# idiap/IdiapTTS

Hardware: AMD Instinct MI355X
Metric: acoustic frames/sec (train) (higher is better)
Workload: dtype f32

## Files before the change

### idiaptts_amd/csrc/sparse_rows.hip

```cpp
#include <algorithm>
#include <atomic>
#include <utility>

#include "activations.h"
#include "common.h"

namespace itts {

constexpr int kSparseMaxK = 512;
constexpr int kSlabCols = 64;
constexpr int kFwdWaves = 16;
constexpr int kRowsPerWave = 4;
constexpr int kStep = 8;
constexpr int kFetch = 16;

static std::atomic<int64_t> g_sparse_path[3];

struct ListLayout {
  int64_t counts_off, entries_off, pitch, bytes;
};

static ListLayout list_layout(int64_t M, int K) {
  ListLayout l;
  l.counts_off = 16;
  l.entries_off = 16 + (M * 4 + 15) / 16 * 16;
  l.pitch = ((int64_t)K + kFetch - 1) / kFetch * kFetch;
  l.bytes = l.entries_off + M * l.pitch * 8;
  return l;
}

__global__ __launch_bounds__(256) void sparse_rows_build_kernel(const uint32_t* __restrict__ x, int64_t ldx, int64_t M,
                                                                int K, int* __restrict__ counts,
                                                                int2* __restrict__ entries, int64_t pitch,
                                                                unsigned long long* __restrict__ record) {
  const int lane = threadIdx.x & 63;
  const int64_t w0 = (int64_t)blockIdx.x * 4 + (threadIdx.x >> 6), wn = (int64_t)gridDim.x * 4;
  const unsigned long long below = (1ull << lane) - 1ull;
  unsigned long long total = 0, most = 0;
  for (int64_t m = w0; m < M; m += wn) {
    const uint32_t* row = x + m * ldx;
    int2* out = entries + m * pitch;
    int cnt = 0;
    for (int k0 = 0; k0 < K; k0 += 256) {
      uint32_t bits[4];
#pragma unroll
      for (int u = 0; u < 4; ++u) {
        const int k = k0 + 64 * u + lane;
        bits[u] = k < K ? row[k] : 0u;
      }
#pragma unroll
      for (int u = 0; u < 4; ++u) {
        const bool nz = (bits[u] & 0x7fffffffu) != 0u;
        const unsigned long long mask = __ballot(nz);
        if (nz) out[cnt + __popcll(mask & below)] = make_int2(k0 + 64 * u + lane, (int)bits[u]);
        cnt += __popcll(mask);
      }
    }
    if (lane < ((kStep - cnt % kStep) % kStep)) out[cnt + lane] = make_int2(K, 0);
    if (lane == 0) counts[m] = cnt;
    total += (unsigned long long)cnt;
    most = std::max(most, (unsigned long long)cnt);
  }
  if (record && lane == 0 && total) {
    atomicAdd(&record[0], total);
    atomicMax(&record[1], most);
  }
}

template <int J>
__device__ __forceinline__ void walk_slot(const float4* slab4, int i16, int2 e, float4& acc) {
  const int k = __builtin_amdgcn_update_dpp(0, e.x, 0x150 + J, 0xf, 0xf, false);
  const float v = __int_as_float(__builtin_amdgcn_update_dpp(0, e.y, 0x150 + J, 0xf, 0xf, false));
  const float4 wk = slab4[k * (kSlabCols / 4) + i16];
  acc.x = fmaf(v, wk.x, acc.x); acc.y = fmaf(v, wk.y, acc.y);
  acc.z = fmaf(v, wk.z, acc.z); acc.w = fmaf(v, wk.w, acc.w);
}
template <int FIRST, int... U>
__device__ __forceinline__ void walk_trip(const float4* slab4, int i16, int2 e, float4& acc,
                                          std::integer_sequence<int, U...>) {
  (walk_slot<FIRST + U>(slab4, i16, e, acc), ...);
}

template <int AF>
__global__ __launch_bounds__(kFwdWaves * 64) void sparse_linear_fwd_kernel(
    const int* __restrict__ counts, const int2* __restrict__ entries, int64_t pitch, const float* __restrict__ w,
    const float* __restrict__ bias, float* __restrict__ y, int64_t ldy, int64_t M, int N, int K, int act, int ranges,
    int store_cols, int wide_out) {
  extern __shared__ float4 slab4[];
  float* slab = reinterpret_cast<float*>(slab4);
  const int lane = threadIdx.x & 63;
  const int wave = __builtin_amdgcn_readfirstlane((int)(threadIdx.x >> 6));
  const int n0 = (int)(blockIdx.x / ranges) * kSlabCols;
  const int range = (int)(blockIdx.x % ranges);
  const int64_t per = (M + ranges - 1) / ranges;
  const int64_t m_begin = range * per, m_end = std::min<int64_t>(M, m_begin + per);
  const int q = lane >> 4, c4 = (lane & 15) * 4;

  {
    const bool col_ok = n0 + lane < N;
    const float* wr = w + (int64_t)(col_ok ? n0 + lane : 0) * K;
    for (int k = wave; k < K; k += kFwdWaves) slab[k * kSlabCols + lane] = col_ok ? wr[k] : 0.f;
    if (wave == 0) slab[K * kSlabCols + lane] = 0.f;
  }

  auto row_of = [&](int64_t group) { return m_begin + (group * kRowsPerWave + q); };
  const int i16 = lane & 15;
  auto fetch = [&](int64_t m, int j0) { return entries[std::min<int64_t>(m, M - 1) * pitch + (j0 + i16)]; };
  int64_t group = wave;
  int2 first = fetch(row_of(group), 0);
  int cnt_next = counts[std::min<int64_t>(row_of(group), M - 1)];
  __syncthreads();

  float4 bv = make_float4(0.f, 0.f, 0.f, 0.f);
  const int n = n0 + c4;
  if (bias) {
    if (n < N) bv.x = bias[n];
    if (n + 1 < N) bv.y = bias[n + 1];
    if (n + 2 < N) bv.z = bias[n + 2];
    if (n + 3 < N) bv.w = bias[n + 3];
  }
  const bool vec_store = wide_out && n + 4 <= store_cols;
  const int last_fetch = (int)pitch - kFetch;

  for (; m_begin + group * kRowsPerWave < m_end; group += kFwdWaves) {
    const int64_t m = row_of(group);
    const int cnt = m < m_end ? cnt_next : 0;
    int2 cur = first;
    first = fetch(row_of(group + kFwdWaves), 0);
    cnt_next = counts[std::min<int64_t>(row_of(group + kFwdWaves), M - 1)];
    int longest = std::max(cnt, __shfl_xor(cnt, 16, 64));
    longest = __builtin_amdgcn_readfirstlane(std::max(longest, __shfl_xor(longest, 32, 64)));
    float4 acc = make_float4(0.f, 0.f, 0.f, 0.f);
    for (int j0 = 0; j0 < longest; j0 += kFetch) {
      const int2 nxt = fetch(m, std::min(j0 + kFetch, last_fetch));
      if (j0 < cnt) walk_trip<0>(slab4, i16, cur, acc, std::make_integer_sequence<int, kStep>());
      if (j0 + kStep < cnt) walk_trip<kStep>(slab4, i16, cur, acc, std::make_integer_sequence<int, kStep>());
      cur = nxt;
    }
    if (m < m_end) {
      float4 o;
      o.x = n < N ? act_fwd_af<AF>(acc.x + bv.x, act) : 0.f;
      o.y = n + 1 < N ? act_fwd_af<AF>(acc.y + bv.y, act) : 0.f;
      o.z = n + 2 < N ? act_fwd_af<AF>(acc.z + bv.z, act) : 0.f;
      o.w = n + 3 < N ? act_fwd_af<AF>(acc.w + bv.w, act) : 0.f;
      float* yr = y + m * ldy + n;
      if (vec_store) {
        *reinterpret_cast<float4*>(yr) = o;
      } else {
        if (n < store_cols) yr[0] = o.x;
        if (n + 1 < store_cols) yr[1] = o.y;
        if (n + 2 < store_cols) yr[2] = o.z;
        if (n + 3 < store_cols) yr[3] = o.w;
      }
    }
  }
}

}

using namespace itts;

extern "C" int itts_sparse_rows_layout(int64_t M, int K, int64_t out[4]) {
  ITTS_REQUIRE(out != nullptr, "null pointer");
  ITTS_REQUIRE(M >= 0 && K > 0 && K <= 65535, "bad sizes (K <= 65535)");
  const ListLayout l = list_layout(M, K);
  out[0] = l.counts_off; out[1] = l.entries_off; out[2] = l.pitch; out[3] = l.bytes;
  return ITTS_OK;
}

extern "C" int itts_sparse_rows_build(const float* d_x, int64_t ldx, int64_t M, int K, void* d_lists, int want_record,
                                      void* stream) {
  ITTS_REQUIRE(d_lists && (M == 0 || d_x), "null pointer");
  ITTS_REQUIRE(M >= 0 && K > 0 && K <= 65535 && ldx >= K, "bad sizes (K <= 65535)");
  ITTS_REQUIRE(aligned16(d_lists), "the list block must be 16-byte aligned");
  hipStream_t s = as_stream(stream);
  char* base = static_cast<char*>(d_lists);
  if (want_record) ITTS_HIP_CHECK(hipMemsetAsync(base, 0, 16, s));
  if (M == 0) return ITTS_OK;
  const ListLayout l = list_layout(M, K);
  const unsigned grid = (unsigned)std::min<int64_t>((M + 3) / 4, 8192);
  hipLaunchKernelGGL(sparse_rows_build_kernel, dim3(grid), dim3(256), 0, s, reinterpret_cast<const uint32_t*>(d_x), ldx,
                     M, K, reinterpret_cast<int*>(base + l.counts_off), reinterpret_cast<int2*>(base + l.entries_off),
                     l.pitch, want_record ? reinterpret_cast<unsigned long long*>(base) : nullptr);
  ITTS_LAUNCH_CHECK();
  g_sparse_path[0].fetch_add(1, std::memory_order_relaxed);
  return ITTS_OK;
}

static int fwd_compute_units() {
  static int cus = 0;
  if (cus == 0) {
    int dev = 0, n = 0;
    if (hipGetDevice(&dev) != hipSuccess ||
        hipDeviceGetAttribute(&n, hipDeviceAttributeMultiprocessorCount, dev) != hipSuccess || n <= 0)
      n = 256;
    cus = n;
  }
  return cus;
}

template <int AF>
static int launch_sparse_fwd(const void* d_lists, const float* d_w, const float* d_b, float* d_y, int64_t ldy, int64_t M,
                             int N, int K, int act, hipStream_t s) {
  static bool lds_set = false;
  if (!lds_set) {
    ITTS_HIP_CHECK(hipFuncSetAttribute((const void*)sparse_linear_fwd_kernel<AF>,
                                       hipFuncAttributeMaxDynamicSharedMemorySize,
                                       (kSparseMaxK + 1) * kSlabCols * 4));
    lds_set = true;
  }
  const ListLayout l = list_layout(M, K);
  const char* base = static_cast<const char*>(d_lists);
  const int slabs = (N + kSlabCols - 1) / kSlabCols;
  const int64_t ranges = std::max<int64_t>(1, std::min<int64_t>(fwd_compute_units() / slabs, (M + 63) / 64));
  const bool wide_out = (ldy % 4 == 0) && aligned16(d_y);
  const int store_cols = wide_out ? (int)std::min<int64_t>((N + 3) / 4 * 4, ldy) : N;
  hipLaunchKernelGGL(sparse_linear_fwd_kernel<AF>, dim3((unsigned)(slabs * ranges)), dim3(kFwdWaves * 64),
                     (size_t)(K + 1) * kSlabCols * 4, s, reinterpret_cast<const int*>(base + l.counts_off),
                     reinterpret_cast<const int2*>(base + l.entries_off), l.pitch, d_w, d_b, d_y, ldy, M, N, K, act,
                     (int)ranges, store_cols, wide_out ? 1 : 0);
  ITTS_LAUNCH_CHECK();
  return ITTS_OK;
}

extern "C" int itts_linear_fwd_sparse(const void* d_lists, const float* d_x, int64_t ldx, const float* d_w,
                                      const float* d_b, float* d_y, int64_t ldy, int64_t M, int N, int K, int act,
                                      void* stream) {
  ITTS_REQUIRE(d_w && (M == 0 || (d_lists && d_x && d_y)), "null pointer");
  ITTS_REQUIRE(M >= 0 && N > 0 && K > 0 && K <= 65535 && ldx >= K && ldy >= N, "bad sizes");
  ITTS_REQUIRE(act >= ITTS_ACT_NONE && act <= ITTS_ACT_HARDSIGMOID, "unknown activation");
  if (M == 0) return ITTS_OK;
  if (K > kSparseMaxK) {
    g_sparse_path[2].fetch_add(1, std::memory_order_relaxed);
    return itts_linear_fwd(d_x, ldx, d_w, d_b, d_y, ldy, M, N, K, act, stream);
  }
  g_sparse_path[1].fetch_add(1, std::memory_order_relaxed);
  if (act_family(act) == AF_EXT) return launch_sparse_fwd<AF_EXT>(d_lists, d_w, d_b, d_y, ldy, M, N, K, act, as_stream(stream));
  return launch_sparse_fwd<AF_BASE>(d_lists, d_w, d_b, d_y, ldy, M, N, K, act, as_stream(stream));
}

extern "C" int itts_sparse_path_counts(int64_t out[3]) {
  ITTS_REQUIRE(out != nullptr, "null pointer");
  for (int i = 0; i < 3; ++i) out[i] = g_sparse_path[i].load(std::memory_order_relaxed);
  return ITTS_OK;
}
```

### idiaptts_amd/csrc/sparse_wgrad.hip

```cpp
#include <algorithm>
#include <atomic>

#include "common.h"

namespace itts {

constexpr int kWgMaxK = 512;
constexpr int kTile = 256;
constexpr int kSlab = 64;
constexpr int kWgWaves = 16;
constexpr int kOwners = 64;
constexpr int kSlots = 8;
constexpr int kStrip = 32;
constexpr int kBlock = 16;
constexpr int kGroup = 4;
constexpr int kHeaderBytes = kSlots * 2;
constexpr int kFirstBytes = kBlock * 8;
constexpr int kOverBytes = (kTile / kBlock - 1) * kBlock * 8;
constexpr int kPlanInv = kStrip + kOwners * kSlots;
constexpr int kPlanInts = kPlanInv + kWgMaxK;
constexpr int kHeavyCode = 0x1000;
constexpr int kRowBytes = kSlab * 4;
constexpr int kBufBytes = (kTile + 1) * kRowBytes;
constexpr int kTPitch = 513;
constexpr int kBiasFloat = 2 * kBufBytes / 4;
constexpr int kWgLdsBytes = 2 * kBufBytes + kSlab * 4;
static_assert(kSlab * kTPitch * 4 <= 2 * kBufBytes, "the output tile reuses the dz buffers");

static std::atomic<int64_t> g_wgrad_path[3];

struct ColsLayout {
  int64_t tiles, strip_off, streams_off, bytes;
};

static ColsLayout cols_layout(int64_t M) {
  ColsLayout l;
  l.tiles = (M + kTile - 1) / kTile;
  l.strip_off = 0;
  l.streams_off = l.tiles * kTile * kStrip * 4;
  l.bytes = l.streams_off + l.tiles * kOwners * (int64_t)(kHeaderBytes + kSlots * (kFirstBytes + kOverBytes));
  return l;
}

__device__ __forceinline__ const char* firsts_of(const char* streams, int tiles) {
  return streams + (int64_t)tiles * kOwners * kHeaderBytes;
}
__device__ __forceinline__ const char* overs_of(const char* streams, int tiles) {
  return firsts_of(streams, tiles) + (int64_t)tiles * kOwners * kSlots * kFirstBytes;
}
__device__ __forceinline__ int2* entry_of(char* streams, int tiles, int64_t pair, int j) {
  char* p = j < kBlock ? const_cast<char*>(firsts_of(streams, tiles)) + pair * kFirstBytes + j * 8
                       : const_cast<char*>(overs_of(streams, tiles)) + pair * kOverBytes + (j - kBlock) * 8;
  return reinterpret_cast<int2*>(p);
}

__global__ __launch_bounds__(256) void sparse_cols_build_kernel(const uint32_t* __restrict__ x, int64_t ldx, int64_t M,
                                                                int K, int parts, int tiles,
                                                                const int* __restrict__ plan,
                                                                uint32_t* __restrict__ strip,
                                                                char* __restrict__ streams) {
  __shared__ int cnts[4][64];
  const int tile = (int)(blockIdx.x / (parts + 1)), part = (int)(blockIdx.x % (parts + 1));
  const int lane = threadIdx.x & 63, wave = threadIdx.x >> 6;
  const int64_t m0 = (int64_t)tile * kTile + wave * 64;
  if (part == parts) {
    const int h = lane & 31;
    const int hc = h < kStrip - 1 ? plan[h] : -1;
    if (!(hc >= 0 && hc < K)) {
      for (int i = 0; i < 32; ++i) {
        const int64_t m = m0 + 2 * i + (lane >> 5);
        strip[m * kStrip + h] = (m < M && h == kStrip - 1) ? 0x3f800000u : 0u;
      }
    }
    for (int pair = threadIdx.x; pair < kOwners * kSlots; pair += 256) {
      const int c = plan[kStrip + pair];
      if (!(c >= 0 && c < K))
        reinterpret_cast<uint16_t*>(streams + ((int64_t)tile * kOwners + pair / kSlots) * kHeaderBytes)[pair % kSlots] = 0;
    }
    return;
  }
  const int k = part * 64 + lane;
  const bool valid = k < K;
  const int code = valid ? plan[kPlanInv + k] : -1;
  const bool light = code >= 0 && code < kOwners * kSlots;
  const bool heavy = code >= kHeavyCode && code < kHeavyCode + kStrip - 1;
  uint32_t bits[64];
#pragma unroll
  for (int r = 0; r < 64; ++r) bits[r] = (valid && m0 + r < M) ? x[(m0 + r) * ldx + k] : 0u;
  int cnt = 0;
#pragma unroll
  for (int r = 0; r < 64; ++r) cnt += (bits[r] & 0x7fffffffu) != 0u ? 1 : 0;
  cnts[wave][lane] = cnt;
  __syncthreads();
  if (heavy) {
    uint32_t* dst = strip + m0 * kStrip + (code - kHeavyCode);
#pragma unroll
    for (int r = 0; r < 64; ++r) dst[r * kStrip] = bits[r];
  }
  if (!light) return;
  int before = 0, total = 0;
#pragma unroll
  for (int w = 0; w < 4; ++w) {
    const int c = cnts[w][lane];
    before += w < wave ? c : 0;
    total += c;
  }
  const int owner = code / kSlots, slot = code % kSlots;
  const int64_t pair = ((int64_t)tile * kOwners + owner) * kSlots + slot;
  int j = before;
#pragma unroll
  for (int r = 0; r < 64; ++r)
    if ((bits[r] & 0x7fffffffu) != 0u)
      *entry_of(streams, tiles, pair, j++) = make_int2((wave * 64 + r) * kRowBytes, (int)bits[r]);
  if (wave == 0) {
    const int end = (total + kBlock - 1) / kBlock * kBlock;
    for (int e = total; e < end; ++e) *entry_of(streams, tiles, pair, e) = make_int2(kTile * kRowBytes, 0);
    reinterpret_cast<uint16_t*>(streams + ((int64_t)tile * kOwners + owner) * kHeaderBytes)[slot] = (uint16_t)total;
  }
}

typedef float floatx16 __attribute__((ext_vector_type(16)));

template <int J>
__device__ __forceinline__ void col_slot(const char* buf, int lane_off, int2 e, float4& acc) {
  const int off = __builtin_amdgcn_update_dpp(0, e.x, 0x150 + J, 0xf, 0xf, false);
  const float v = __int_as_float(__builtin_amdgcn_update_dpp(0, e.y, 0x150 + J, 0xf, 0xf, false));
  const float4 d = *reinterpret_cast<const float4*>(buf + off + lane_off);
  acc.x = fmaf(v, d.x, acc.x); acc.y = fmaf(v, d.y, acc.y);
  acc.z = fmaf(v, d.z, acc.z); acc.w = fmaf(v, d.w, acc.w);
}
template <int FIRST>
__device__ __forceinline__ void col_group(const char* buf, int lane_off, int2 e, float4& acc) {
  col_slot<FIRST>(buf, lane_off, e, acc);
  col_slot<FIRST + 1>(buf, lane_off, e, acc);
  col_slot<FIRST + 2>(buf, lane_off, e, acc);
  col_slot<FIRST + 3>(buf, lane_off, e, acc);
}

__global__ __launch_bounds__(kWgWaves * 64) void sparse_wgrad_kernel(
    const float* __restrict__ dz, int64_t lddz, const float* __restrict__ strip, const char* __restrict__ streams,
    const int* __restrict__ plan, float* __restrict__ slabs, int64_t slab_stride, int lddw,
    float* __restrict__ bias_part, int64_t bias_stride, int64_t M, int N, int K, int tiles, int per, int ranges) {
  extern __shared__ float4 smem4[];
  char* smem = reinterpret_cast<char*>(smem4);
  float* smemf = reinterpret_cast<float*>(smem4);
  const int tid = threadIdx.x, lane = tid & 63;
  const int wave = __builtin_amdgcn_readfirstlane(tid >> 6);
  const int i16 = lane & 15, owner = wave * 4 + (lane >> 4);
  const int n0 = (int)(blockIdx.x / ranges) * kSlab;
  const int range = (int)(blockIdx.x % ranges);
  const int t_begin = range * per, t_end = std::min(tiles, t_begin + per);

  if (tid < 128) smemf[((tid >> 6) * kBufBytes + kTile * kRowBytes) / 4 + lane] = 0.f;

  const int srow = tid >> 4, c4 = (tid & 15) * 4, n = n0 + c4;
  auto load_tile = [&](int t, float4 (&st)[4]) {
#pragma unroll
    for (int p = 0; p < 4; ++p) {
      const int64_t m = (int64_t)t * kTile + p * 64 + srow;
      float4 v = make_float4(0.f, 0.f, 0.f, 0.f);
      if (m < M) {
        const float* src = dz + m * lddz + n;
        if (n + 4 <= N) {
          v = *reinterpret_cast<const float4*>(src);
        } else {
          if (n < N) v.x = src[0];
          if (n + 1 < N) v.y = src[1];
          if (n + 2 < N) v.z = src[2];
        }
      }
      st[p] = v;
    }
  };
  auto store_tile = [&](int b, const float4 (&st)[4]) {
#pragma unroll
    for (int p = 0; p < 4; ++p)
      *reinterpret_cast<float4*>(smem + b * kBufBytes + (p * 64 + srow) * kRowBytes + c4 * 4) = st[p];
  };
  const char* firsts = firsts_of(streams, tiles) + i16 * 8;
  const char* overs = overs_of(streams, tiles) + i16 * 8;
  auto lists_of = [&](int t) { return ((int64_t)t * kOwners + owner) * kSlots; };

  float4 acc[kSlots];
#pragma unroll
  for (int c = 0; c < kSlots; ++c) acc[c] = make_float4(0.f, 0.f, 0.f, 0.f);
  floatx16 hacc;
#pragma unroll
  for (int r = 0; r < 16; ++r) hacc[r] = 0.f;

  uint4 hdr;
  int2 first[kSlots];
  auto load_lists = [&](int t) {
    hdr = *reinterpret_cast<const uint4*>(streams + ((int64_t)t * kOwners + owner) * kHeaderBytes);
#pragma unroll
    for (int c = 0; c < kSlots; ++c)
      first[c] = *reinterpret_cast<const int2*>(firsts + (lists_of(t) + c) * kFirstBytes);
  };
  auto count_of = [&](int c) {
    const uint32_t word = c < 2 ? hdr.x : (c < 4 ? hdr.y : (c < 6 ? hdr.z : hdr.w));
    return (int)((word >> ((c & 1) * 16)) & 0xffffu);
  };

  float4 st[4];
  load_tile(t_begin, st);
  load_lists(t_begin);
  store_tile(0, st);
  __syncthreads();

  const int hb = wave >> 3, hr0 = (wave & 7) * 32 + (lane >> 5);
  for (int t = t_begin; t < t_end; ++t) {
    const int b = (t - t_begin) & 1;
    const int tn = std::min(t + 1, t_end - 1);
    const char* buf = smem + b * kBufBytes;
    const char* more = overs + lists_of(t) * kOverBytes;
    int2 over = first[0];
    if (count_of(0) > kBlock) over = *reinterpret_cast<const int2*>(more);
#pragma unroll
    for (int c = 0; c < kSlots; ++c) {
      const int cnt = count_of(c);
      int longest = std::max(cnt, __shfl_xor(cnt, 16, 64));
      longest = __builtin_amdgcn_readfirstlane(std::max(longest, __shfl_xor(longest, 32, 64)));
      int2 over_n = over;
      if (c + 1 < kSlots && count_of(c + 1 < kSlots ? c + 1 : c) > kBlock)
        over_n = *reinterpret_cast<const int2*>(more + (c + 1) * kOverBytes);
      int2 cur = first[c];
      for (int j0 = 0; j0 < longest; j0 += kBlock) {
        const int left = cnt - j0;
        if (left > 0) {
          int2 ahead = over;
          if (left > 2 * kBlock) ahead = *reinterpret_cast<const int2*>(more + c * kOverBytes + (j0 + kBlock) * 8);
          col_group<0>(buf, i16 * 16, cur, acc[c]);
          if (left > kGroup) col_group<kGroup>(buf, i16 * 16, cur, acc[c]);
          if (left > 2 * kGroup) col_group<2 * kGroup>(buf, i16 * 16, cur, acc[c]);
          if (left > 3 * kGroup) col_group<3 * kGroup>(buf, i16 * 16, cur, acc[c]);
          cur = over;
          over = ahead;
        }
      }
      over = over_n;
    }
    load_tile(tn, st);
    {
      const float* a = reinterpret_cast<const float*>(buf) + hr0 * kSlab + hb * 32 + (lane & 31);
      const float* xh = strip + ((int64_t)t * kTile + hr0) * kStrip + (lane & 31);
#pragma unroll
      for (int kk = 0; kk < 16; ++kk)
        hacc = __builtin_amdgcn_mfma_f32_32x32x2f32(a[2 * kk * kSlab], xh[2 * kk * kStrip], hacc, 0, 0, 0);
    }
    store_tile(b ^ 1, st);
    load_lists(tn);
    __syncthreads();
  }

  for (int i = tid; i < kBiasFloat + kSlab; i += kWgWaves * 64) smemf[i] = 0.f;
  __syncthreads();
#pragma unroll
  for (int c = 0; c < kSlots; ++c) {
    const int col = plan[kStrip + owner * kSlots + c];
    if (col >= 0 && col < K) {
      smemf[(4 * i16 + 0) * kTPitch + col] = acc[c].x;
      smemf[(4 * i16 + 1) * kTPitch + col] = acc[c].y;
      smemf[(4 * i16 + 2) * kTPitch + col] = acc[c].z;
      smemf[(4 * i16 + 3) * kTPitch + col] = acc[c].w;
    }
  }
  __syncthreads();
  {
    const int h = lane & 31;
    const int hc = h < kStrip - 1 ? plan[h] : -1;
    for (int w = 0; w < kWgWaves; ++w) {
      if (wave == w) {
#pragma unroll
        for (int r = 0; r < 16; ++r) {
          const int nl = hb * 32 + 8 * (r / 4) + 4 * (lane >> 5) + (r % 4);
          if (h == kStrip - 1) smemf[kBiasFloat + nl] += hacc[r];
          else if (hc >= 0 && hc < K) smemf[nl * kTPitch + hc] += hacc[r];
        }
      }
      __syncthreads();
    }
  }
  for (int nn = wave; nn < kSlab; nn += kWgWaves) {
    if (n0 + nn < N) {
      float* dst = slabs + range * slab_stride + (int64_t)(n0 + nn) * lddw;
      for (int k = lane; k < lddw; k += 64) dst[k] = smemf[nn * kTPitch + k];
    }
  }
  if (bias_part && tid < kSlab && n0 + tid < N)
    bias_part[range * bias_stride + n0 + tid] = smemf[kBiasFloat + tid];
}

static int wgrad_compute_units() {
  static int cus = 0;
  if (cus == 0) {
    int dev = 0, n = 0;
    if (hipGetDevice(&dev) != hipSuccess ||
        hipDeviceGetAttribute(&n, hipDeviceAttributeMultiprocessorCount, dev) != hipSuccess || n <= 0)
      n = 256;
    cus = n;
  }
  return cus;
}

static void wgrad_ranges(int64_t M, int N, int* per, int* ranges) {
  const int64_t tiles = (M + kTile - 1) / kTile;
  const int slabs = (N + kSlab - 1) / kSlab;
  const int64_t want = std::max<int64_t>(1, std::min<int64_t>(wgrad_compute_units() / slabs, tiles));
  *per = (int)((tiles + want - 1) / want);
  *ranges = (int)((tiles + *per - 1) / *per);
}

static bool wgrad_shape_ok(int K, int64_t lddw) { return K <= kWgMaxK && lddw <= kWgMaxK; }

}

using namespace itts;

extern "C" int itts_sparse_cols_plan_ints(void) { return kPlanInts; }

extern "C" int itts_sparse_cols_layout(int64_t M, int K, int64_t out[3]) {
  ITTS_REQUIRE(out != nullptr, "null pointer");
  ITTS_REQUIRE(M >= 0 && K > 0 && K <= kWgMaxK, "bad sizes (K <= 512)");
  const ColsLayout l = cols_layout(M);
  out[0] = l.strip_off; out[1] = l.streams_off; out[2] = l.bytes;
  return ITTS_OK;
}

extern "C" int itts_sparse_cols_build(const float* d_x, int64_t ldx, int64_t M, int K, const int* d_plan, void* d_cols,
                                      void* stream) {
  ITTS_REQUIRE(d_plan && d_cols && (M == 0 || d_x), "null pointer");
  ITTS_REQUIRE(M >= 0 && K > 0 && K <= kWgMaxK && ldx >= K, "bad sizes (K <= 512)");
  ITTS_REQUIRE(aligned16(d_cols), "the column block must be 16-byte aligned");
  if (M == 0) return ITTS_OK;
  const ColsLayout l = cols_layout(M);
  const int parts = (K + 63) / 64;
  ITTS_REQUIRE(l.tiles * (parts + 1) < ((int64_t)1 << 31), "too many rows");
  char* base = static_cast<char*>(d_cols);
  hipLaunchKernelGGL(sparse_cols_build_kernel, dim3((unsigned)(l.tiles * (parts + 1))), dim3(256), 0,
                     as_stream(stream), reinterpret_cast<const uint32_t*>(d_x), ldx, M, K, parts, (int)l.tiles, d_plan,
                     reinterpret_cast<uint32_t*>(base + l.strip_off), base + l.streams_off);
  ITTS_LAUNCH_CHECK();
  g_wgrad_path[0].fetch_add(1, std::memory_order_relaxed);
  return ITTS_OK;
}

extern "C" int64_t itts_linear_bwd_weight_sparse_workspace_bytes(int64_t M, int N, int K, int64_t lddw) {
  if (M < 0 || N <= 0 || K <= 0 || lddw < K) return 0;
  const int64_t dense = itts_linear_bwd_weight_workspace_bytes(M, N, (int)lddw);
  if (M == 0 || !wgrad_shape_ok(K, lddw)) return dense;
  int per, ranges;
  wgrad_ranges(M, N, &per, &ranges);
  return std::max<int64_t>(dense, (int64_t)ranges * ((int64_t)N * lddw + N) * 4);
}

extern "C" int itts_linear_bwd_weight_sparse(const float* d_dz, int64_t lddz, const void* d_cols, const int* d_plan,
                                             const float* d_x, int64_t ldx, float* d_dw, int64_t lddw, float* d_db,
                                             int64_t M, int N, int K, void* d_workspace, int accumulate,
                                             void* stream) {
  ITTS_REQUIRE(d_dw && d_workspace && (M == 0 || (d_dz && d_x)), "null pointer");
  ITTS_REQUIRE(M >= 0 && N > 0 && K > 0 && lddz >= N && ldx >= K && lddw >= K, "bad sizes");
  ITTS_REQUIRE(lddw == K || ldx >= lddw, "x must be as wide as dw's rows (its pad columns zero)");
  const bool sparse = M > 0 && d_cols && d_plan && wgrad_shape_ok(K, lddw) && lddz % 4 == 0 && aligned16(d_dz) &&
                      aligned16(d_cols);
  if (!sparse) {
    if (M > 0) g_wgrad_path[2].fetch_add(1, std::memory_order_relaxed);
    return itts_linear_bwd_weight(d_dz, lddz, d_x, ldx, d_dw, d_db, M, N, (int)lddw, d_workspace, accumulate, stream);
  }
  hipStream_t s = as_stream(stream);
  static bool lds_set = false;
  if (!lds_set) {
    ITTS_HIP_CHECK(hipFuncSetAttribute((const void*)sparse_wgrad_kernel, hipFuncAttributeMaxDynamicSharedMemorySize,
                                       kWgLdsBytes));
    lds_set = true;
  }
  const ColsLayout l = cols_layout(M);
  int per, ranges;
  wgrad_ranges(M, N, &per, &ranges);
  const int slabs_n = (N + kSlab - 1) / kSlab;
  ITTS_REQUIRE((int64_t)slabs_n * ranges < ((int64_t)1 << 31), "too many workgroups");
  const int64_t n = (int64_t)N * lddw;
  const bool merged = d_db && d_db == d_dw + n && N % 4 == 0 && n % 4 == 0;
  float* ws = static_cast<float*>(d_workspace);
  float* bias_part = !d_db ? nullptr : (merged ? ws + n : ws + (int64_t)ranges * n);
  const char* base = static_cast<const char*>(d_cols);
  hipLaunchKernelGGL(sparse_wgrad_kernel, dim3((unsigned)(slabs_n * ranges)), dim3(kWgWaves * 64), kWgLdsBytes, s, d_dz,
                     lddz, reinterpret_cast<const float*>(base + l.strip_off), base + l.streams_off, d_plan, ws,
                     merged ? n + N : n, (int)lddw, bias_part, merged ? n + N : (int64_t)N, M, N, K, (int)l.tiles, per,
                     ranges);
  ITTS_LAUNCH_CHECK();
  g_wgrad_path[1].fetch_add(1, std::memory_order_relaxed);
  if (merged) return reduce_slabs(ws, ranges, n + N, d_dw, accumulate, s);
  int rc = reduce_slabs(ws, ranges, n, d_dw, accumulate, s);
  if (rc || !d_db) return rc;
  return reduce_slabs(bias_part, ranges, (int64_t)N, d_db, accumulate, s);
}

extern "C" int itts_sparse_wgrad_counts(int64_t out[3]) {
  ITTS_REQUIRE(out != nullptr, "null pointer");
  for (int i = 0; i < 3; ++i) out[i] = g_wgrad_path[i].load(std::memory_order_relaxed);
  return ITTS_OK;
}
```

Baseline: 41.02 million.

## Vectorize sparse forward weight slab fill and parallelize wgrad hidden-tile reduction

The sparse forward kernel now loads weight rows as float4 when K is a multiple of four and the pointer is 16-byte aligned, then scatters the four values into the transposed LDS slab. The wgrad kernel replaces a sixteen-step serialized per-wave accumulation, which had a barrier per wave, with a staged LDS reduction. In that reduction each wave stores its MFMA accumulators, then sums two rows across the eight waves of its half-block and writes the result directly. This removes many block-wide barriers at the cost of extra LDS traffic and an assumption about how the hb groups are laid out across waves.

```diff
diff --git a/idiaptts_amd/csrc/sparse_rows.hip b/idiaptts_amd/csrc/sparse_rows.hip
--- a/idiaptts_amd/csrc/sparse_rows.hip
+++ b/idiaptts_amd/csrc/sparse_rows.hip
@@ -13,6 +13,7 @@
 constexpr int kRowsPerWave = 4;
 constexpr int kStep = 8;
 constexpr int kFetch = 16;
+constexpr int kFillTrips = kSparseMaxK / 4 / kFwdWaves;
 
 static std::atomic<int64_t> g_sparse_path[3];
 
@@ -85,7 +86,7 @@
 __global__ __launch_bounds__(kFwdWaves * 64) void sparse_linear_fwd_kernel(
     const int* __restrict__ counts, const int2* __restrict__ entries, int64_t pitch, const float* __restrict__ w,
     const float* __restrict__ bias, float* __restrict__ y, int64_t ldy, int64_t M, int N, int K, int act, int ranges,
-    int store_cols, int wide_out) {
+    int store_cols, int wide_out, int wide_w) {
   extern __shared__ float4 slab4[];
   float* slab = reinterpret_cast<float*>(slab4);
   const int lane = threadIdx.x & 63;
@@ -99,7 +100,26 @@
   {
     const bool col_ok = n0 + lane < N;
     const float* wr = w + (int64_t)(col_ok ? n0 + lane : 0) * K;
-    for (int k = wave; k < K; k += kFwdWaves) slab[k * kSlabCols + lane] = col_ok ? wr[k] : 0.f;
+    if (wide_w) {
+      const float4* wr4 = reinterpret_cast<const float4*>(wr);
+      const int K4 = K >> 2;
+      float4 v[kFillTrips];
+#pragma unroll
+      for (int u = 0; u < kFillTrips; ++u) {
+        const int j = wave + u * kFwdWaves;
+        v[u] = (col_ok && j < K4) ? wr4[j] : make_float4(0.f, 0.f, 0.f, 0.f);
+      }
+#pragma unroll
+      for (int u = 0; u < kFillTrips; ++u) {
+        const int j = wave + u * kFwdWaves;
+        if (j < K4) {
+          float* row = slab + 4 * j * kSlabCols + lane;
+          row[0] = v[u].x; row[kSlabCols] = v[u].y; row[2 * kSlabCols] = v[u].z; row[3 * kSlabCols] = v[u].w;
+        }
+      }
+    } else {
+      for (int k = wave; k < K; k += kFwdWaves) slab[k * kSlabCols + lane] = col_ok ? wr[k] : 0.f;
+    }
     if (wave == 0) slab[K * kSlabCols + lane] = 0.f;
   }
 
@@ -218,7 +238,7 @@
   hipLaunchKernelGGL(sparse_linear_fwd_kernel<AF>, dim3((unsigned)(slabs * ranges)), dim3(kFwdWaves * 64),
                      (size_t)(K + 1) * kSlabCols * 4, s, reinterpret_cast<const int*>(base + l.counts_off),
                      reinterpret_cast<const int2*>(base + l.entries_off), l.pitch, d_w, d_b, d_y, ldy, M, N, K, act,
-                     (int)ranges, store_cols, wide_out ? 1 : 0);
+                     (int)ranges, store_cols, wide_out ? 1 : 0, (K % 4 == 0 && aligned16(d_w)) ? 1 : 0);
   ITTS_LAUNCH_CHECK();
   return ITTS_OK;
 }
diff --git a/idiaptts_amd/csrc/sparse_wgrad.hip b/idiaptts_amd/csrc/sparse_wgrad.hip
--- a/idiaptts_amd/csrc/sparse_wgrad.hip
+++ b/idiaptts_amd/csrc/sparse_wgrad.hip
@@ -252,6 +252,22 @@
     __syncthreads();
   }
 
+  float hsum[2];
+  {
+#pragma unroll
+    for (int r = 0; r < 16; ++r) smemf[(wave * 16 + r) * 64 + lane] = hacc[r];
+    __syncthreads();
+#pragma unroll
+    for (int rr = 0; rr < 2; ++rr) {
+      const int r = 2 * (wave & 7) + rr;
+      float s = 0.f;
+#pragma unroll
+      for (int w = 0; w < 8; ++w) s += smemf[((hb * 8 + w) * 16 + r) * 64 + lane];
+      hsum[rr] = s;
+    }
+    __syncthreads();
+  }
+
   for (int i = tid; i < kBiasFloat + kSlab; i += kWgWaves * 64) smemf[i] = 0.f;
   __syncthreads();
 #pragma unroll
@@ -264,22 +280,18 @@
       smemf[(4 * i16 + 3) * kTPitch + col] = acc[c].w;
     }
   }
-  __syncthreads();
   {
     const int h = lane & 31;
     const int hc = h < kStrip - 1 ? plan[h] : -1;
-    for (int w = 0; w < kWgWaves; ++w) {
-      if (wave == w) {
-#pragma unroll
-        for (int r = 0; r < 16; ++r) {
-          const int nl = hb * 32 + 8 * (r / 4) + 4 * (lane >> 5) + (r % 4);
-          if (h == kStrip - 1) smemf[kBiasFloat + nl] += hacc[r];
-          else if (hc >= 0 && hc < K) smemf[nl * kTPitch + hc] += hacc[r];
-        }
-      }
-      __syncthreads();
-    }
-  }
+#pragma unroll
+    for (int rr = 0; rr < 2; ++rr) {
+      const int r = 2 * (wave & 7) + rr;
+      const int nl = hb * 32 + 8 * (r / 4) + 4 * (lane >> 5) + (r % 4);
+      if (h == kStrip - 1) smemf[kBiasFloat + nl] = hsum[rr];
+      else if (hc >= 0 && hc < K) smemf[nl * kTPitch + hc] = hsum[rr];
+    }
+  }
+  __syncthreads();
   for (int nn = wave; nn < kSlab; nn += kWgWaves) {
     if (n0 + nn < N) {
       float* dst = slabs + range * slab_stride + (int64_t)(n0 + nn) * lddw;
```

New measurement: 42.12 million (median of 6 runs). 1.03x the previous value.
